# velocyto-team/velocyto.py

Hardware: AMD Instinct MI355X
Metric: cells/sec through knn_imputation->fit_slope->colDeltaCor, 50k cells x 30k genes (higher is better)
Workload: dtype f64

## Files before the change

### velocyto.py_amd/csrc/coldeltacor.hip

```cpp
#include <stdlib.h>
#include "common.h"
#ifndef VCY_EXP
#define VCY_EXP 0
#endif
#include <type_traits>

namespace vcy {

template <typename T> __device__ __forceinline__ T fast_sqrt(T x);
template <> __device__ __forceinline__ float fast_sqrt<float>(float x) { return __builtin_amdgcn_sqrtf(x); }
template <> __device__ __forceinline__ double fast_sqrt<double>(double x) { return sqrt(x); }
template <typename T> __device__ __forceinline__ T fast_log10(T x);
template <> __device__ __forceinline__ float fast_log10<float>(float x) { return __builtin_amdgcn_logf(x) * 0.30102999566398120f; }
template <> __device__ __forceinline__ double fast_log10<double>(double x) { return log10(x); }

template <typename T, int TR, int RULES> __device__ __forceinline__ T xform(T t, T psc)
{
    if (TR == VCY_LINEAR) return t;
    const T a = fabs(t) + psc;
    const T s = (TR == VCY_SQRT) ? fast_sqrt<T>(a) : fast_log10<T>(a);
    if (TR == VCY_SQRT && RULES != VCY_RULES_FULL)
        return (fabs(t) < T(1e-16)) ? T(0) : copysign(s, t);
    T r;
    if (TR == VCY_LOG10 && RULES == VCY_RULES_PARTIAL) r = (t >= T(0)) ? s : -s;
    else r = (t > T(0)) ? s : -s;
    return r;
}

template <> __device__ __forceinline__ float xform<float, VCY_SQRT, VCY_RULES_PARTIAL>(float t, float psc)
{
    const float c = __builtin_amdgcn_fmed3f(fabsf(t) * 0x1p54f, 0.0f, 1.0f);
    return copysignf(fast_sqrt<float>(fmaf(psc, c, fabsf(t))), t);
}

template <> __device__ __forceinline__ double xform<double, VCY_SQRT, VCY_RULES_PARTIAL_ROOT2>(double t, double psc)
{
    const double x = fabs(t) + psc;
    const float xf0 = (float)x;
    const float xf = (fabs(t) < 1e-16) ? __builtin_inff() : xf0;
    const float yf = __builtin_amdgcn_rsqf(xf);
    const double s0 = (double)(xf0 * yf), h = (double)(0.5f * yf);
    double d = fma(-s0, s0, x);
    const double s1 = fma(d, h, s0);
    d = fma(-s1, s1, x);
    return copysign(fma(d, h, s1), t);
}

template <> __device__ __forceinline__ double xform<double, VCY_SQRT, VCY_RULES_PARTIAL>(double t, double psc)
{
    const double x = fabs(t) + psc;
    const float xf0 = (float)x;
    const float xf = (fabs(t) < 1e-16) ? __builtin_inff() : xf0;
    const double y = (double)__builtin_amdgcn_rsqf(xf);
    const double u = x * y;
    return copysign(u * fma(-u, y, 3.0), t);
}

extern "C" __device__ float vcy_fmul_legacy(float, float) __asm("llvm.amdgcn.fmul.legacy");
template <> __device__ __forceinline__ float xform<float, VCY_SQRT, VCY_RULES_PARTIAL_NOPSC>(float t, float)
{
    return vcy_fmul_legacy(t, __builtin_amdgcn_rsqf(fabsf(t)));
}

template <int TR, int RULES> struct Shifted { static constexpr bool value = TR == VCY_LOG10 || (TR == VCY_SQRT && RULES == VCY_RULES_FULL); };

template <typename T, int TR, int RULES> struct ZeroMasked {
    static constexpr bool value = std::is_same<T, double>::value && TR == VCY_SQRT && (RULES == VCY_RULES_PARTIAL || RULES == VCY_RULES_PARTIAL_ROOT2);
};
template <int RULES> __device__ __forceinline__ double xform_kept(double t, double psc)
{
    const double x = fabs(t) + psc;
    const float xf = (float)x;
    const float yf = __builtin_amdgcn_rsqf(xf);
    if constexpr (RULES == VCY_RULES_PARTIAL_ROOT2) {
        const double s0 = (double)(xf * yf), h = (double)(0.5f * yf);
        double d = fma(-s0, s0, x);
        const double s1 = fma(d, h, s0);
        d = fma(-s1, s1, x);
        return copysign(fma(d, h, s1), t);
    } else {
        const double y = (double)yf;
        const double u = x * y;
        return copysign(u * fma(-u, y, 3.0), t);
    }
}

template <typename T, int TR, int RULES> __device__ __forceinline__ T xform_shift(T psc)
{
    if (!Shifted<TR, RULES>::value) return T(0);
    const T k = xform<T, TR, RULES>(T(0), psc);
    return (k - k == T(0)) ? k : T(0);
}
template <> __device__ __forceinline__ float xform_shift<float, VCY_LOG10, VCY_RULES_PARTIAL>(float psc)
{
    const float l0 = __builtin_amdgcn_logf(psc);
    return (l0 - l0 == 0.f) ? l0 : 0.f;
}
template <> __device__ __forceinline__ float xform_shift<float, VCY_LOG10, VCY_RULES_FULL>(float psc)
{
    const float l0 = -__builtin_amdgcn_logf(psc);
    return (l0 - l0 == 0.f) ? l0 : 0.f;
}

template <typename T, int TR, int RULES> __device__ __forceinline__ T xform_s(T t, T psc, T K)
{
    const T a = xform<T, TR, RULES>(t, psc);
    return Shifted<TR, RULES>::value ? a - K : a;
}
template <> __device__ __forceinline__ float xform_s<float, VCY_LOG10, VCY_RULES_PARTIAL>(float t, float psc, float K)
{
    const float l = __builtin_amdgcn_logf(fabsf(t) + psc);
    return (((t >= 0.f) ? l : -l) - K) * 0.30102999566398120f;
}
template <> __device__ __forceinline__ float xform_s<float, VCY_LOG10, VCY_RULES_FULL>(float t, float psc, float K)
{
    const float l = __builtin_amdgcn_logf(fabsf(t) + psc);
    return (((t > 0.f) ? l : -l) - K) * 0.30102999566398120f;
}

template <typename T> __device__ __forceinline__ T pearson_from_moments(double sA, double sAA, double sAb, double sb, double sbb, double n)
{
    if (n < 2.0) return (T)__builtin_nan("");
    const double cov = sAb - sA * sb / n;
    const double va = sAA - sA * sA / n;
    const double vb = sbb - sb * sb / n;
    return (T)(cov / sqrt(va * vb));
}

template <typename T> struct FuseArgs {
    const T *Ux;
    const float *gamma, *q;
    T dt_shift, used_dt;
};

template <typename T, int TR> __device__ __forceinline__ T fused_dmat(T s, T u, float gm, float qq, T dt_shift, T used_dt, T psc)
{
    const T upred = (T)gm * s + (T)qq;
    const T ds = dt_shift * (u - upred);
    const T D = (s + used_dt * ds) - s;
    if (TR == VCY_LINEAR) return D;
    const T a = fabs(D) + psc;
    const T f = (TR == VCY_SQRT) ? fast_sqrt<T>(a) : fast_log10<T>(a);
    return D > T(0) ? f : (D < T(0) ? -f : T(0) * f);
}

template <typename T, int TR, int RULES>
__global__ __launch_bounds__(1024) void k_cdc_partial(const T *__restrict__ e, const T *__restrict__ d,
                                                       const int32_t *__restrict__ ixs, T *__restrict__ out,
                                                       const int32_t *__restrict__ order, int G, int64_t ld,
                                                       int64_t cell0, int64_t d_row0, int C_out, int nrndm, int gchunk, T psc, FuseArgs<T> fuse)
{
    using V = typename Vec<T>::type;
    constexpr int N = Vec<T>::N;
    constexpr int UNROLL = 4;
    extern __shared__ __attribute__((aligned(16))) char smem[];
    T *ec = reinterpret_cast<T *>(smem);
    T *dc = ec + gchunk;
    T *acc = dc + gchunk;
    double *red = reinterpret_cast<double *>(acc + 3 * ((nrndm + 1) & ~1));

    const int tid = threadIdx.x, lane = tid & 63, wave = tid >> 6, nwaves = blockDim.x >> 6;
    const int per_x = (C_out + 7) / 8;
    const int pos = ((int)blockIdx.x & 7) * per_x + ((int)blockIdx.x >> 3);
    if (pos >= C_out) return;
    const int cl = order ? order[pos] : pos;
    const int64_t c = cell0 + cl;
    const T *erow_c = e + c * ld;
    const T *drow_c = (fuse.Ux ? fuse.Ux : d) + (c - d_row0) * ld;

    for (int n = tid; n < 3 * nrndm; n += blockDim.x) acc[n] = T(0);
    double sb = 0.0, sbb = 0.0;
    const T K = xform_shift<T, TR, RULES>(psc);

    for (int g0 = 0; g0 < G; g0 += gchunk) {
        const int gl = min(gchunk, G - g0);
        const int nvec = gl / N;
        __syncthreads();
        for (int v = tid; v < nvec; v += blockDim.x) {
            const V ev = reinterpret_cast<const V *>(erow_c + g0)[v];
            V dv = reinterpret_cast<const V *>(drow_c + g0)[v];
            if (fuse.Ux) {
                const T *ep = reinterpret_cast<const T *>(&ev);
                T *dq = reinterpret_cast<T *>(&dv);
#pragma unroll
                for (int k = 0; k < N; ++k) {
                    const int g = g0 + v * N + k;
                    dq[k] = fused_dmat<T, TR>(ep[k], dq[k], fuse.gamma[g], fuse.q ? fuse.q[g] : 0.f, fuse.dt_shift, fuse.used_dt, psc);
                }
            }
            reinterpret_cast<V *>(ec)[v] = ev;
            reinterpret_cast<V *>(dc)[v] = dv;
            const T *dp = reinterpret_cast<const T *>(&dv);
#pragma unroll
            for (int k = 0; k < N; ++k) { sb += (double)dp[k]; sbb += (double)dp[k] * (double)dp[k]; }
        }
        for (int g = nvec * N + tid; g < gl; g += blockDim.x) {
            const T ev = erow_c[g0 + g];
            T dv = drow_c[g0 + g];
            if (fuse.Ux) dv = fused_dmat<T, TR>(ev, dv, fuse.gamma[g0 + g], fuse.q ? fuse.q[g0 + g] : 0.f, fuse.dt_shift, fuse.used_dt, psc);
            ec[g] = ev; dc[g] = dv;
            sb += (double)dv; sbb += (double)dv * (double)dv;
        }
        __syncthreads();

        for (int n = wave; n < nrndm; n += nwaves) {
            const int i = __builtin_amdgcn_readfirstlane(ixs[(int64_t)cl * nrndm + n]);
            const T *row = e + (int64_t)i * ld + g0;
            T sA[N], sAA[N], sAb[N];
#pragma unroll
            for (int k = 0; k < N; ++k) { sA[k] = T(0); sAA[k] = T(0); sAb[k] = T(0); }
            int v = lane;
            for (; v + 64 * (UNROLL - 1) < nvec; v += 64 * UNROLL) {
                V x[UNROLL];
#pragma unroll
                for (int u = 0; u < UNROLL; ++u) x[u] = reinterpret_cast<const V *>(row)[v + 64 * u];
#pragma unroll
                for (int u = 0; u < UNROLL; ++u) {
                    const V ecv = reinterpret_cast<const V *>(ec)[v + 64 * u];
                    const V dcv = reinterpret_cast<const V *>(dc)[v + 64 * u];
                    const T *xp = reinterpret_cast<const T *>(&x[u]);
                    const T *ep = reinterpret_cast<const T *>(&ecv);
                    const T *bp = reinterpret_cast<const T *>(&dcv);
#pragma unroll
                    for (int k = 0; k < N; ++k) {
                        const T tt = xp[k] - ep[k];
                        T a = xform_s<T, TR, RULES>(tt, psc, K);
                        sA[k] += a;
                        if (RULES == VCY_RULES_PARTIAL_NOPSC) sAA[k] += fabs(tt);
                        else sAA[k] = fma(a, a, sAA[k]);
                        sAb[k] = fma(a, bp[k], sAb[k]);
                    }
                }
            }
            for (; v < nvec; v += 64) {
                const V xv = reinterpret_cast<const V *>(row)[v];
                const V ecv = reinterpret_cast<const V *>(ec)[v];
                const V dcv = reinterpret_cast<const V *>(dc)[v];
                const T *xp = reinterpret_cast<const T *>(&xv);
                const T *ep = reinterpret_cast<const T *>(&ecv);
                const T *bp = reinterpret_cast<const T *>(&dcv);
#pragma unroll
                for (int k = 0; k < N; ++k) {
                    const T tt = xp[k] - ep[k];
                    T a = xform_s<T, TR, RULES>(tt, psc, K);
                    sA[k] += a;
                    if (RULES == VCY_RULES_PARTIAL_NOPSC) sAA[k] += fabs(tt);
                    else sAA[k] = fma(a, a, sAA[k]);
                    sAb[k] = fma(a, bp[k], sAb[k]);
                }
            }
            {
                const int g = nvec * N + lane;
                if (g < gl) {
                    const T tt = row[g] - ec[g];
                    T a = xform_s<T, TR, RULES>(tt, psc, K);
                    sA[0] += a;
                    if (RULES == VCY_RULES_PARTIAL_NOPSC) sAA[0] += fabs(tt);
                    else sAA[0] = fma(a, a, sAA[0]);
                    sAb[0] = fma(a, dc[g], sAb[0]);
                }
            }
            T tA = sA[0], tAA = sAA[0], tAb = sAb[0];
#pragma unroll
            for (int k = 1; k < N; ++k) { tA += sA[k]; tAA += sAA[k]; tAb += sAb[k]; }
            tA = wave_sum(tA); tAA = wave_sum(tAA); tAb = wave_sum(tAb);
            if (lane == 0) {
                acc[3 * n + 0] += tA;
                acc[3 * n + 1] += tAA;
                acc[3 * n + 2] += tAb;
            }
        }
    }
    sb = block_sum(sb, red);
    sbb = block_sum(sbb, red);
    for (int n = tid; n < nrndm; n += blockDim.x)
        out[(int64_t)cl * nrndm + n] = pearson_from_moments<T>((double)acc[3 * n], (double)acc[3 * n + 1],
                                                               (double)acc[3 * n + 2], sb, sbb, (double)G);
}

constexpr int GRP_NV = 6;
constexpr int GRP_GC_DUAL = 6, GRP_NV_DUAL = 6;
constexpr int GRP_GC = 8;
constexpr int GRP_GC_F64 = 6, GRP_NV_F64 = 8;
constexpr int GRP_GC_DUAL_F64 = 4;

template <typename T> __host__ __device__ inline size_t grouped_lds_bytes(int gc, int nv, bool dual, int64_t maxpairs, int npad)
{
    const int as = dual ? 4 : 3;
    return (size_t)(dual ? 3 : 2) * gc * nv * 64 * 16 + (size_t)npad * 8 + sizeof(T) * (size_t)as * ((maxpairs + 1) & ~(int64_t)1) +
           8 * (size_t)(maxpairs + 2 > 64 + 4 * gc ? maxpairs + 2 : 64 + 4 * gc) + (size_t)(gc + 18) * sizeof(int) + 16;
}

template <int K, bool FULL> struct RowVecs { static constexpr int value = K; static constexpr bool full = FULL; };
template <int K, int NV, typename F> __device__ __forceinline__ void for_even_count(int n, F &f)
{
    if constexpr (K + 2 <= NV) {
        if (n == K) f(RowVecs<K, false>{});
        else for_even_count<K + 2, NV>(n, f);
    } else
        f(RowVecs<K, false>{});
}

template <typename T, int TR, int RULES, int GC, int NV, bool DUAL>
__global__ __launch_bounds__(1024) void k_cdc_partial_grouped(const T *__restrict__ e, const T *__restrict__ d, const T *__restrict__ d2,
                                                               const int32_t *__restrict__ ixs, T *__restrict__ out, T *__restrict__ out2,
                                                               const int32_t *__restrict__ order, int G, int64_t ld, int64_t cell0,
                                                               int64_t d_row0, int C_main, int tile_main, int C_tail, int tile_tail, int nrndm_all, int stride, int npad, T psc,
                                                               FuseArgs<T> fuse)
{
    using V = typename Vec<T>::type;
    constexpr int N = Vec<T>::N;
    constexpr int GCHUNK = NV * 64 * N;
    constexpr int AS = DUAL ? 4 : 3;
    constexpr int PW = DUAL ? 4 : 2;
    extern __shared__ __attribute__((aligned(16))) char smem[];
    const int maxpairs = GC * max(tile_main, tile_tail);
    T *ec = reinterpret_cast<T *>(smem);
    T *dc = ec + GC * GCHUNK;
    T *dc2 = dc + GC * GCHUNK;
    unsigned long long *keys = reinterpret_cast<unsigned long long *>(dc + (DUAL ? 2 : 1) * GC * GCHUNK);
    T *acc = reinterpret_cast<T *>(keys + npad);
    unsigned long long *desc = reinterpret_cast<unsigned long long *>(acc + AS * ((maxpairs + 1) & ~1));
    double *part = reinterpret_cast<double *>(desc);
    double *s_sb = part + 64, *s_sbb = s_sb + GC, *s_sb2 = s_sbb + GC, *s_sbb2 = s_sb2 + GC;
    int *s_cells = reinterpret_cast<int *>(desc + max(maxpairs + 2, 64 + 4 * GC));
    int *s_wavetot = s_cells + GC;
    int &s_U = s_wavetot[16];
    int *s_next = s_wavetot + 17;

    const int tid = threadIdx.x, lane = tid & 63, wave = tid >> 6, nwaves = blockDim.x >> 6;
    const int nb_main = ((((C_main + GC - 1) / GC) + 7) / 8 * 8) * (C_main > 0 ? (nrndm_all + tile_main - 1) / tile_main : 0);
    const bool tail = (int)blockIdx.x >= nb_main;
    const int bx = tail ? (int)blockIdx.x - nb_main : (int)blockIdx.x;
    const int C_out = tail ? C_tail : C_main, pos0 = tail ? C_main : 0, tilew = tail ? tile_tail : tile_main;
    const int ngroups = (C_out + GC - 1) / GC, per = (ngroups + 7) / 8, gblocks = per * 8;
    const int tile = bx / gblocks, bg = bx - tile * gblocks;
    const int gpos = (bg & 7) * per + (bg >> 3);
    if (gpos >= ngroups) return;
    const int n0 = tile * tilew;
    const int nrndm = min(tilew, nrndm_all - n0);
    ixs += n0;
    out += n0;
    if (DUAL) out2 += n0;
    const int g0cell = gpos * GC;
    const int gcount = min(GC, C_out - g0cell);
    const int npairs = gcount * nrndm;
    if (tid < GC) s_cells[tid] = tid < gcount ? (order ? order[pos0 + g0cell + tid] : pos0 + g0cell + tid) : 0;
    __syncthreads();
    for (int t = tid; t < npad; t += blockDim.x) {
        unsigned long long key = ~0ull;
        if (t < npairs) {
            const int m = t / nrndm, n = t - m * nrndm;
            const unsigned i = (unsigned)ixs[(int64_t)s_cells[m] * stride + n];
            key = ((unsigned long long)i << 16) | ((unsigned long long)m << 12) | (unsigned)n;
        }
        keys[t] = key;
    }
    __syncthreads();
    for (int size = 2; size <= npad; size <<= 1) {
        for (int stride = size >> 1; stride > 0; stride >>= 1) {
            for (int t = tid; t < npad / 2; t += blockDim.x) {
                const int lo = 2 * t - (t & (stride - 1)), hi = lo + stride;
                const bool up = ((lo & size) == 0);
                const unsigned long long a = keys[lo], b = keys[hi];
                if ((a > b) == up) { keys[lo] = b; keys[hi] = a; }
            }
            __syncthreads();
        }
    }
    {
        static_assert(GC <= 8, "member mask is 8 bits");
        auto head = [&](int t) {
            if (t == 0) return true;
            const unsigned long long a = keys[t] >> 12, b = keys[t - 1] >> 12;
            return (a >> 4) != (b >> 4) || a == b;
        };
        const int per = (npad + blockDim.x - 1) / blockDim.x;
        const int t0 = tid * per, t1 = min(npairs, t0 + per);
        int cnt = 0;
        for (int t = t0; t < t1; ++t) cnt += head(t) ? 1 : 0;
        int incl = cnt;
#pragma unroll
        for (int off = 1; off < 64; off <<= 1) { const int o = __shfl_up(incl, off, 64); if (lane >= off) incl += o; }
        if (lane == 63) s_wavetot[wave] = incl;
        __syncthreads();
        int base = 0;
        for (int w = 0; w < wave; ++w) base += s_wavetot[w];
        int rank = base + incl - cnt;
        for (int t = t0; t < t1; ++t)
            if (head(t)) {
                unsigned mask = 0;
                int q = t;
                do { mask |= 1u << (unsigned)((keys[q] >> 12) & 15); ++q; } while (q < npairs && !head(q));
                desc[rank++] = ((keys[t] >> 16) << 19) | ((unsigned long long)mask << 11) | (unsigned)t;
            }
        if (tid == blockDim.x - 1) { s_U = base + incl; }
        __syncthreads();
    }
    for (int t = tid; t < AS * npairs; t += blockDim.x) acc[t] = T(0);
    __syncthreads();
    const int U = s_U;
    const T K = xform_shift<T, TR, RULES>(psc);
    const int sm = wave % GC, sh = wave / GC, snh = max(1, nwaves / GC);
    double psb = 0.0, psbb = 0.0, psb2 = 0.0, psbb2 = 0.0;

    for (int g0 = 0; g0 < G; g0 += GCHUNK) {
        const int gl = min(GCHUNK, G - g0);
        const int nvec = (gl + N - 1) / N;
        const bool ragged = (gl % N) != 0;
        const int nvu = min(NV, ((nvec + 63) / 64 + 1) & ~1);
        __syncthreads();
        if (tid == 0) *s_next = 0;
        if (sh < snh && sm < gcount) {
            const int64_t c = cell0 + s_cells[sm];
            const T *er = e + c * ld + g0;
            const T *dr = (fuse.Ux ? fuse.Ux : d) + (c - d_row0) * ld + g0;
            const T *dr2 = DUAL ? d2 + (c - d_row0) * ld + g0 : nullptr;
            for (int v = sh * 64 + lane; v < nvec; v += 64 * snh) {
                V ev = reinterpret_cast<const V *>(er)[v];
                V dv = reinterpret_cast<const V *>(dr)[v];
                V dv2;
                if (DUAL) dv2 = reinterpret_cast<const V *>(dr2)[v];
                T *dp = reinterpret_cast<T *>(&dv);
                T *dp2 = reinterpret_cast<T *>(&dv2);
                T *ep = reinterpret_cast<T *>(&ev);
                if (fuse.Ux) {
#pragma unroll
                    for (int k = 0; k < N; ++k) {
                        const int g = g0 + v * N + k;
                        if (g < G) dp[k] = fused_dmat<T, TR>(ep[k], dp[k], fuse.gamma[g], fuse.q ? fuse.q[g] : 0.f, fuse.dt_shift, fuse.used_dt, psc);
                    }
                }
                if (ragged && v == nvec - 1) {
#pragma unroll
                    for (int k = 0; k < N; ++k) if (k >= gl - v * N) { dp[k] = T(0); ep[k] = T(0); if (DUAL) dp2[k] = T(0); }
                }
                reinterpret_cast<V *>(ec + sm * GCHUNK)[v] = ev;
                reinterpret_cast<V *>(dc + sm * GCHUNK)[v] = dv;
                if (DUAL) reinterpret_cast<V *>(dc2 + sm * GCHUNK)[v] = dv2;
#pragma unroll
                for (int k = 0; k < N; ++k) {
                    psb += (double)dp[k]; psbb += (double)dp[k] * (double)dp[k];
                    if (DUAL) { psb2 += (double)dp2[k]; psbb2 += (double)dp2[k] * (double)dp2[k]; }
                }
            }
        }
        if (gl < GCHUNK && sh < snh && sm < gcount)
            for (int v = nvec + sh * 64 + lane; v < nvu * 64; v += 64 * snh) {
                reinterpret_cast<V *>(ec + sm * GCHUNK)[v] = V{};
                reinterpret_cast<V *>(dc + sm * GCHUNK)[v] = V{};
                if (DUAL) reinterpret_cast<V *>(dc2 + sm * GCHUNK)[v] = V{};
            }
        __syncthreads();
        static_assert(NV % 2 == 0, "operand buffers alternate");
#define VCY_FENCE() __builtin_amdgcn_sched_barrier(0)
        auto load_row = [&](auto nvc, V (&x)[NV], unsigned long long dsc) {
            constexpr int KV = decltype(nvc)::value;
            const T *row = e + (int64_t)(dsc >> 19) * ld + g0;
#pragma unroll
            for (int u = 0; u < KV; ++u) {
                const int v = lane + 64 * u;
                if (decltype(nvc)::full || v < nvec) x[u] = reinterpret_cast<const V *>(row)[v];
                else x[u] = V{};
            }
        };
        auto eval_row = [&](auto nvc, const V (&x)[NV], unsigned long long dsc) {
            constexpr int KV = decltype(nvc)::value;
            int p = (int)(dsc & 2047);
            unsigned mask = (unsigned)(dsc >> 11) & 255u;
            int m = __builtin_ctz(mask);
            constexpr int RD = 2;
            static_assert(KV % RD == 0, "operand buffers rotate");
            V eR[RD], bR[RD], b2R[RD];
            auto rd = [&](V &ev, V &bv, V &b2v, int mm, int u) {
                ev = reinterpret_cast<const V *>(ec + mm * GCHUNK)[lane + 64 * u];
                bv = reinterpret_cast<const V *>(dc + mm * GCHUNK)[lane + 64 * u];
                if (DUAL) b2v = reinterpret_cast<const V *>(dc2 + mm * GCHUNK)[lane + 64 * u];
            };
#pragma unroll
            for (int u = 0; u < RD - 1; ++u) rd(eR[u], bR[u], b2R[u], m, u);
            while (mask) {
                mask &= mask - 1;
                const int mn = mask ? __builtin_ctz(mask) : m;
                T sA, sAA, sAb, sAb2;
                constexpr bool MASKED = ZeroMasked<T, TR, RULES>::value;
                if constexpr (MASKED) { sA = sAA = sAb = T(0); if (DUAL) sAb2 = T(0); }
                auto fold = [&](const V &xv, const V &ev, const V &bv, const V &b2v, bool first) {
                    const T *xp = reinterpret_cast<const T *>(&xv);
                    const T *ep = reinterpret_cast<const T *>(&ev);
                    const T *bp = reinterpret_cast<const T *>(&bv);
                    const T *bp2 = reinterpret_cast<const T *>(&b2v);
                    constexpr bool ABS2 = RULES == VCY_RULES_PARTIAL_NOPSC;
#pragma unroll
                    for (int k = 0; k < N; ++k) {
                        const T tt = xp[k] - ep[k];
                        if constexpr (MASKED) {
                            if (!(fabs(tt) < 1e-16)) {
                                const T a = xform_kept<RULES>(tt, psc);
                                sA += a;
                                sAA = fma(a, a, sAA);
                                sAb = fma(a, bp[k], sAb);
                                if (DUAL) sAb2 = fma(a, bp2[k], sAb2);
                            }
                            continue;
                        }
                        const T a = xform_s<T, TR, RULES>(tt, psc, K);
                        if (first && k == 0) {
                            sA = a;
                            sAA = ABS2 ? fabs(tt) : a * a;
                            sAb = a * bp[k];
                            if (DUAL) sAb2 = a * bp2[k];
                            continue;
                        }
                        sA += a;
                        if (ABS2) sAA += fabs(tt);
                        else sAA = fma(a, a, sAA);
                        sAb = fma(a, bp[k], sAb);
                        if (DUAL) sAb2 = fma(a, bp2[k], sAb2);
                    }
                };
#pragma unroll
                for (int u = 0; u < KV; ++u) {
                    constexpr int AHEAD = RD - 1;
                    const int un = u + AHEAD;
                    if (un < KV) rd(eR[un % RD], bR[un % RD], b2R[un % RD], m, un);
                    else rd(eR[un % RD], bR[un % RD], b2R[un % RD], mn, un - KV);
                    VCY_FENCE();
                    fold(x[u], eR[u % RD], bR[u % RD], b2R[u % RD], u == 0);
                    VCY_FENCE();
                }
                const T tot = wave_sum_rows_quads(sA, sAA, sAb, DUAL ? sAb2 : T(0));
                if ((lane & 3) == 0 && (lane >> 4) < AS)
                    __hip_atomic_fetch_add(&acc[AS * p + (lane >> 4)], tot, __ATOMIC_RELAXED, __HIP_MEMORY_SCOPE_WORKGROUP);
                ++p;
                m = mn;
            }
        };
        auto rows = [&](auto nvc) {
            auto ticket = [&]() { int t = 0; if (lane == 0) t = atomicAdd(s_next, 1); return t; };
            auto uni = [&](unsigned long long v) {
                const unsigned lo = (unsigned)__builtin_amdgcn_readfirstlane((int)(unsigned)v);
                const unsigned hi = (unsigned)__builtin_amdgcn_readfirstlane((int)(unsigned)(v >> 32));
                return ((unsigned long long)hi << 32) | lo;
            };
            constexpr int TAIL = 64;
            const int U4 = U > TAIL ? ((U - TAIL) & ~3) : 0, T4 = U4 >> 2;
            auto first_row = [&](int v) { return v < T4 ? 4 * v : U4 + 2 * (v - T4); };
            V xa[NV], xb[NV];
            int v = __builtin_amdgcn_readfirstlane(ticket());
            int q = min(first_row(v), U);
            unsigned long long w0 = 0, w1 = 0, w2 = 0, w3 = 0;
            if (q < U) { w0 = uni(desc[q]); w1 = uni(desc[min(q + 1, U - 1)]); w2 = uni(desc[min(q + 2, U - 1)]); w3 = uni(desc[min(q + 3, U - 1)]); }
            if (q < U) load_row(nvc, xa, w0);
            while (v < T4) {
                const int tv = ticket();
                load_row(nvc, xb, w1);
                eval_row(nvc, xa, w0);
                load_row(nvc, xa, w2);
                eval_row(nvc, xb, w1);
                const int vn = __builtin_amdgcn_readfirstlane(tv);
                const int qn = min(first_row(vn), U);
                unsigned long long n0 = 0, n1 = 0, n2 = 0, n3 = 0;
                if (qn < U) { n0 = desc[qn]; n1 = desc[min(qn + 1, U - 1)]; n2 = desc[min(qn + 2, U - 1)]; n3 = desc[min(qn + 3, U - 1)]; }
                load_row(nvc, xb, w3);
                eval_row(nvc, xa, w2);
                if (qn < U) { n0 = uni(n0); n1 = uni(n1); n2 = uni(n2); n3 = uni(n3); }
                if (qn < U) load_row(nvc, xa, n0);
                eval_row(nvc, xb, w3);
                v = vn; q = qn; w0 = n0; w1 = n1; w2 = n2; w3 = n3;
            }
            while (q < U) {
                const int tv = ticket();
                const bool two = q + 1 < U;
                if (two) load_row(nvc, xb, w1);
                eval_row(nvc, xa, w0);
                const int vn = __builtin_amdgcn_readfirstlane(tv);
                const int qn = min(first_row(vn), U);
                unsigned long long n0 = 0, n1 = 0;
                if (qn < U) { n0 = uni(desc[qn]); n1 = uni(desc[min(qn + 1, U - 1)]); }
                if (qn < U) load_row(nvc, xa, n0);
                if (two) eval_row(nvc, xb, w1);
                v = vn; q = qn; w0 = n0; w1 = n1;
            }
        };
        if (nvec == 64 * NV) rows(RowVecs<NV, true>{});
        else for_even_count<2, NV>(nvu, rows);
    }
    psb = wave_sum(psb); psbb = wave_sum(psbb);
    if (DUAL) { psb2 = wave_sum(psb2); psbb2 = wave_sum(psbb2); }
    __syncthreads();
    if (lane == 0) {
        part[PW * wave] = psb; part[PW * wave + 1] = psbb;
        if (DUAL) { part[PW * wave + 2] = psb2; part[PW * wave + 3] = psbb2; }
    }
    __syncthreads();
    if (tid < gcount) {
        double a = 0.0, b = 0.0, a2 = 0.0, b2 = 0.0;
        for (int h = 0; h < snh; ++h) {
            const int w = tid + h * GC;
            if (w < nwaves) { a += part[PW * w]; b += part[PW * w + 1]; if (DUAL) { a2 += part[PW * w + 2]; b2 += part[PW * w + 3]; } }
        }
        s_sb[tid] = a; s_sbb[tid] = b; s_sb2[tid] = a2; s_sbb2[tid] = b2;
    }
    __syncthreads();
    for (int p = tid; p < npairs; p += blockDim.x) {
        const unsigned long long key = keys[p];
        const int m = (int)((key >> 12) & 15), n = (int)(key & 4095);
        const double mA = (double)acc[AS * p], mAA = (double)acc[AS * p + 1];
        out[(int64_t)s_cells[m] * stride + n] = pearson_from_moments<T>(mA, mAA, (double)acc[AS * p + 2], s_sb[m], s_sbb[m], (double)G);
        if (DUAL) out2[(int64_t)s_cells[m] * stride + n] = pearson_from_moments<T>(mA, mAA, (double)acc[AS * p + 3], s_sb2[m], s_sbb2[m], (double)G);
    }
}

constexpr int FULL_TC = 16, FULL_TI = 64, FULL_GK = 32;

template <typename T, int TR>
__global__ __launch_bounds__(256) void k_cdc_full(const T *__restrict__ e, const T *__restrict__ d, T *__restrict__ rm,
                                                   int C, int G, int64_t ld, int64_t cell0, int C_out, int64_t ld_rm,
                                                   T psc, int accumulate)
{
    __shared__ T ei[FULL_TI][FULL_GK + 1];
    __shared__ T ecs[FULL_TC][FULL_GK];
    __shared__ T dcs[FULL_TC][FULL_GK];
    __shared__ double sbs[FULL_TC][2];
    const int tid = threadIdx.x, il = tid & 63, cg = tid >> 6;
    const int i0 = blockIdx.x * FULL_TI, c0 = blockIdx.y * FULL_TC;
    T sA[4], sAA[4], sAb[4];
#pragma unroll
    for (int k = 0; k < 4; ++k) { sA[k] = T(0); sAA[k] = T(0); sAb[k] = T(0); }
    const int sg = tid & 31, sr = tid >> 5;
    double sb = 0.0, sbb = 0.0;
    double sb2 = 0.0, sbb2 = 0.0;
    const T K = xform_shift<T, TR, VCY_RULES_FULL>(psc);
    for (int g0 = 0; g0 < G; g0 += FULL_GK) {
        const int glen = min(FULL_GK, G - g0);
        __syncthreads();
        const bool gok = sg < glen;
#pragma unroll
        for (int r = 0; r < 8; ++r) {
            const int row = sr + 8 * r, gi = i0 + row;
            ei[row][sg] = (gok && gi < C) ? e[(int64_t)gi * ld + g0 + sg] : T(0);
        }
#pragma unroll
        for (int r = 0; r < 2; ++r) {
            const int row = sr + 8 * r;
            const int64_t gc = cell0 + c0 + row;
            const bool ok = gok && (c0 + row) < C_out;
            const T ev = ok ? e[gc * ld + g0 + sg] : T(0);
            const T dv = ok ? d[gc * ld + g0 + sg] : T(0);
            ecs[row][sg] = ev;
            dcs[row][sg] = dv;
            if (r == 0) { sb += (double)dv; sbb += (double)dv * (double)dv; }
            else { sb2 += (double)dv; sbb2 += (double)dv * (double)dv; }
        }
        __syncthreads();
        for (int g = 0; g < glen; ++g) {
            const T x = ei[il][g];
#pragma unroll
            for (int k = 0; k < 4; ++k) {
                T a = xform_s<T, TR, VCY_RULES_FULL>(x - ecs[cg * 4 + k][g], psc, K);
                sA[k] += a;
                sAA[k] = fma(a, a, sAA[k]);
                sAb[k] = fma(a, dcs[cg * 4 + k][g], sAb[k]);
            }
        }
    }
#pragma unroll
    for (int off = 16; off > 0; off >>= 1) {
        sb += __shfl_xor(sb, off, 64); sbb += __shfl_xor(sbb, off, 64);
        sb2 += __shfl_xor(sb2, off, 64); sbb2 += __shfl_xor(sbb2, off, 64);
    }
    if (sg == 0) { sbs[sr][0] = sb; sbs[sr][1] = sbb; sbs[sr + 8][0] = sb2; sbs[sr + 8][1] = sbb2; }
    __syncthreads();
    const int gi = i0 + il;
    if (gi < C) {
#pragma unroll
        for (int k = 0; k < 4; ++k) {
            const int crow = c0 + cg * 4 + k;
            if (crow < C_out) {
                const T r = pearson_from_moments<T>((double)sA[k], (double)sAA[k], (double)sAb[k],
                                                    sbs[cg * 4 + k][0], sbs[cg * 4 + k][1], (double)G);
                T *p = rm + (int64_t)crow * ld_rm + gi;
                *p = accumulate ? (*p + r) : r;
            }
        }
    }
}

template <typename T>
__global__ void k_scatter_rows(const T *__restrict__ vals, const int32_t *__restrict__ ixs, T *__restrict__ rm,
                               int64_t total, int nrndm, int64_t ld_rm)
{
    for (int64_t t = blockIdx.x * (int64_t)blockDim.x + threadIdx.x; t < total; t += (int64_t)gridDim.x * blockDim.x) {
        const int64_t c = t / nrndm;
        atomicAdd(rm + c * ld_rm + ixs[t], vals[t]);
    }
}

template <typename T, int TR, int RULES, int GC, int NV, bool DUAL>
static int launch_grouped(const void *e, const void *d, const void *d2, const int32_t *ixs, void *out, void *out2, const int32_t *order, int64_t G,
                          int64_t ld, int64_t cell0, int64_t C_out, int64_t d_row0, int64_t nrndm, double psc, hipStream_t st,
                          FuseArgs<T> fuse, const DevInfo &dev, bool *done)
{
    constexpr int64_t TILE_MAX = 256;
    static_assert(GC * TILE_MAX <= 2048, "a row descriptor holds the first pair of the row in 11 bits");
    *done = false;
    const size_t budget_g = (size_t)(dev.lds_optin > 163840 ? 163840 : dev.lds_optin);
    int64_t ntiles = (nrndm + TILE_MAX - 1) / TILE_MAX, tile = 0;
    int npad = 2;
    size_t lds_g = 0;
    for (;; ++ntiles) {
        tile = (nrndm + ntiles - 1) / ntiles;
        const int64_t maxpairs = GC * tile;
        for (npad = 2; npad < maxpairs; npad <<= 1) {}
        lds_g = grouped_lds_bytes<T>(GC, NV, DUAL, maxpairs, npad);
        if (lds_g <= budget_g || tile <= 16) break;
    }
    if (!(nrndm >= 8 && C_out >= 4 * GC && nrndm <= 0x7fffffff / 2 && lds_g <= budget_g)) return VCY_OK;
    auto kern = k_cdc_partial_grouped<T, TR, RULES, GC, NV, DUAL>;
    int rc = ensure_dynamic_lds(reinterpret_cast<const void *>(kern), lds_g);
    if (rc) return rc;
    const int64_t groups = (C_out + GC - 1) / GC, W = dev.cus > 0 ? dev.cus : 256;
    const int64_t full = groups >= W ? groups / W * W : 0;
    const int64_t c_main = full * GC, c_tail = C_out - c_main;
    int64_t tw = tile;
    if (c_tail > 0) {
        const int64_t left = groups - full;
        constexpr double OVH = 0.05;
        double best = 0.0;
        int64_t bs = 1;
        for (int64_t s = 1; s == 1 || (tile + s - 1) / s >= 16; ++s) {
            const int64_t w = (tile + s - 1) / s, nt = (nrndm + w - 1) / w;
            const double t = (double)((left * nt + W - 1) / W) * ((double)w / (double)tile + OVH);
            if (s == 1 || t < 0.98 * best) { best = t; bs = s; }
        }
        tw = (tile + bs - 1) / bs;
    }
    auto nblocks = [&](int64_t ncell, int64_t w) { return ncell > 0 ? ((ncell + GC - 1) / GC + 7) / 8 * 8 * ((nrndm + w - 1) / w) : (int64_t)0; };
    hipLaunchKernelGGL(kern, dim3((unsigned)(nblocks(c_main, tile) + nblocks(c_tail, tw))), dim3(1024), lds_g, st, (const T *)e, (const T *)d,
                       (const T *)d2, ixs, (T *)out, (T *)out2, order, (int)G, ld, cell0, d_row0, (int)c_main, (int)tile, (int)c_tail, (int)tw,
                       (int)nrndm, (int)nrndm, npad, (T)psc, fuse);
    VCY_LAUNCH_CHECK();
    *done = true;
    return VCY_OK;
}

template <typename T, int TR, int RULES>
static int launch_partial(const void *e, const void *d, const void *d2, const int32_t *ixs, void *out, void *out2, const int32_t *order, int64_t G,
                          int64_t ld, int64_t cell0, int64_t C_out, int64_t d_row0, int64_t nrndm, double psc, hipStream_t st,
                          FuseArgs<T> fuse = FuseArgs<T>{nullptr, nullptr, nullptr, T(1), T(1)})
{
    constexpr int N = Vec<T>::N;
    DevInfo dev;
    int rc = device_info(&dev);
    if (rc) return rc;
    if (env_int("VCY_CDC_GROUP", GRP_GC) == GRP_GC) {
        bool done = false;
        if (d2) {
            if constexpr (sizeof(T) == 8) {
                if (env_int("VCY_CDC_DUAL_F64", 1) == 1)
                    rc = launch_grouped<T, TR, RULES, GRP_GC_DUAL_F64, GRP_NV_F64, true>(e, d, d2, ixs, out, out2, order, G, ld, cell0, C_out, d_row0, nrndm, psc, st, fuse, dev, &done);
                else
                    rc = launch_grouped<T, TR, RULES, GRP_GC_DUAL, GRP_NV_DUAL, true>(e, d, d2, ixs, out, out2, order, G, ld, cell0, C_out, d_row0, nrndm, psc, st, fuse, dev, &done);
            } else
                rc = launch_grouped<T, TR, RULES, GRP_GC_DUAL, GRP_NV_DUAL, true>(e, d, d2, ixs, out, out2, order, G, ld, cell0, C_out, d_row0, nrndm, psc, st, fuse, dev, &done);
        } else if constexpr (sizeof(T) == 8)
            rc = launch_grouped<T, TR, RULES, GRP_GC_F64, GRP_NV_F64, false>(e, d, nullptr, ixs, out, nullptr, order, G, ld, cell0, C_out, d_row0, nrndm, psc, st, fuse, dev, &done);
        else
            rc = launch_grouped<T, TR, RULES, GRP_GC, GRP_NV, false>(e, d, nullptr, ixs, out, nullptr, order, G, ld, cell0, C_out, d_row0, nrndm, psc, st, fuse, dev, &done);
        if (rc || done) return rc;
    }
    if (d2) {
        rc = launch_partial<T, TR, RULES>(e, d, nullptr, ixs, out, nullptr, order, G, ld, cell0, C_out, d_row0, nrndm, psc, st, fuse);
        if (rc) return rc;
        return launch_partial<T, TR, RULES>(e, d2, nullptr, ixs, out2, nullptr, order, G, ld, cell0, C_out, d_row0, nrndm, psc, st);
    }
    const int quantum = 64 * N;
    const size_t fixed = sizeof(T) * 3 * ((nrndm + 1) & ~1) + 32 * sizeof(double);
    const size_t budget = (size_t)(dev.lds_optin > 153600 ? 153600 : dev.lds_optin);
    if (fixed + 2 * quantum * sizeof(T) > budget)
        return fail(VCY_ERR_UNSUPPORTED, "%s: nrndm=%lld needs more LDS than the %lld-byte budget", "coldeltacor_partial", (long long)nrndm, (long long)budget);
    const int64_t max_chunk = (int64_t)((budget - fixed) / (2 * sizeof(T))) / quantum * quantum;
    const int64_t Gq = (G + quantum - 1) / quantum * quantum;
    const int64_t nchunks = (Gq + max_chunk - 1) / max_chunk;
    int64_t gchunk = ((Gq / quantum + nchunks - 1) / nchunks) * quantum;
    const size_t lds = fixed + 2 * gchunk * sizeof(T);
    auto kern = k_cdc_partial<T, TR, RULES>;
    rc = ensure_dynamic_lds(reinterpret_cast<const void *>(kern), lds);
    if (rc) return rc;
    const int threads = (nrndm >= 16) ? 1024 : (nrndm >= 8 ? 512 : 256);
    hipLaunchKernelGGL(kern, dim3((unsigned)((C_out + 7) / 8 * 8)), dim3(threads), lds, st, (const T *)e, (const T *)d, ixs, (T *)out, order,
                       (int)G, ld, cell0, d_row0, (int)C_out, (int)nrndm, (int)gchunk, (T)psc, fuse);
    VCY_LAUNCH_CHECK();
    return VCY_OK;
}

template <typename T>
static int dispatch_partial(const void *e, const void *d, const void *d2, const int32_t *ixs, void *out, void *out2, const int32_t *order, int64_t G,
                            int64_t ld, int64_t cell0, int64_t C_out, int64_t d_row0, int64_t nrndm, int transform, int rules,
                            double psc, hipStream_t st, FuseArgs<T> fuse = FuseArgs<T>{nullptr, nullptr, nullptr, T(1), T(1)})
{
#define VCY_CASE(TR, RU) \
    if (transform == TR && rules == RU) return launch_partial<T, TR, RU>(e, d, d2, ixs, out, out2, order, G, ld, cell0, C_out, d_row0, nrndm, psc, st, fuse);
    if (rules == VCY_RULES_PARTIAL_ROOT2) {
        if constexpr (std::is_same<T, double>::value) { VCY_CASE(VCY_SQRT, VCY_RULES_PARTIAL_ROOT2) }
        rules = VCY_RULES_PARTIAL;
    }
    VCY_CASE(VCY_LINEAR, VCY_RULES_PARTIAL)
    VCY_CASE(VCY_LINEAR, VCY_RULES_FULL)
    VCY_CASE(VCY_SQRT, VCY_RULES_PARTIAL)
    VCY_CASE(VCY_SQRT, VCY_RULES_FULL)
    VCY_CASE(VCY_LOG10, VCY_RULES_PARTIAL)
    VCY_CASE(VCY_LOG10, VCY_RULES_FULL)
    if constexpr (std::is_same<T, float>::value) { VCY_CASE(VCY_SQRT, VCY_RULES_PARTIAL_NOPSC) }
#undef VCY_CASE
    if (rules == VCY_RULES_PARTIAL_NOPSC) return fail(VCY_ERR_INVALID, "%s: VCY_RULES_PARTIAL_NOPSC is defined for VCY_SQRT on VCY_F32 only", "coldeltacor_partial");
    return fail(VCY_ERR_INVALID, "%s: bad transform/rules", "coldeltacor_partial");
}

template <typename T>
static int dispatch_full(const void *e, const void *d, void *rm, int64_t C, int64_t G, int64_t ld, int64_t cell0,
                         int64_t C_out, int64_t ld_rm, int transform, double psc, int accumulate, hipStream_t st)
{
    dim3 grid((unsigned)((C + FULL_TI - 1) / FULL_TI), (unsigned)((C_out + FULL_TC - 1) / FULL_TC));
#define VCY_CASE(TR)                                                                                                        \
    if (transform == TR) {                                                                                                  \
        hipLaunchKernelGGL((k_cdc_full<T, TR>), grid, dim3(256), 0, st, (const T *)e, (const T *)d, (T *)rm, (int)C, (int)G, \
                           ld, cell0, (int)C_out, ld_rm, (T)psc, accumulate);                                              \
        VCY_LAUNCH_CHECK();                                                                                                 \
        return VCY_OK;                                                                                                      \
    }
    VCY_CASE(VCY_LINEAR)
    VCY_CASE(VCY_SQRT)
    VCY_CASE(VCY_LOG10)
#undef VCY_CASE
    return fail(VCY_ERR_INVALID, "%s: bad transform", "coldeltacor_full");
}

}

using namespace vcy;

static int check_partial_args(const char *who, const void *e, const void *d, const int32_t *ixs, const void *out, int64_t C, int64_t G, int64_t ld,
                              int64_t cell0, int64_t C_out, int64_t d_row0, int64_t nrndm, int dtype)
{
    if (!(e && d && ixs && out)) return fail(VCY_ERR_INVALID, "%s: null pointer", who);
    if (!(C > 0 && G > 0 && nrndm > 0 && C_out > 0 && cell0 >= 0 && cell0 + C_out <= C)) return fail(VCY_ERR_INVALID, "%s: bad shape", who);
    if (ld < G) return fail(VCY_ERR_INVALID, "%s: ld < G", who);
    if (!(d_row0 >= 0 && d_row0 <= cell0)) return fail(VCY_ERR_INVALID, "%s: d must cover cells cell0..cell0+C_out-1", who);
    if (!(dtype == VCY_F32 || dtype == VCY_F64)) return fail(VCY_ERR_INVALID, "%s: bad dtype", who);
    if (ld % (dtype == VCY_F32 ? 4 : 2) != 0) return fail(VCY_ERR_INVALID, "%s: ld must keep rows 16-byte aligned", who);
    if (((uintptr_t)e % 16) || ((uintptr_t)d % 16)) return fail(VCY_ERR_INVALID, "%s: e/d must be 16-byte aligned", who);
    return VCY_OK;
}

extern "C" int vcy_coldeltacor_partial(const void *e, const void *d, const int32_t *ixs, void *out, const int32_t *order,
                                       int64_t C, int64_t G, int64_t ld, int64_t cell0, int64_t C_out, int64_t d_row0,
                                       int64_t nrndm, int transform, int rules, double psc, int dtype, vcy_stream stream)
{
    int rc = check_partial_args("coldeltacor_partial", e, d, ixs, out, C, G, ld, cell0, C_out, d_row0, nrndm, dtype);
    if (rc) return rc;
    hipStream_t st = as_stream(stream);
    if (dtype == VCY_F32) return dispatch_partial<float>(e, d, nullptr, ixs, out, nullptr, order, G, ld, cell0, C_out, d_row0, nrndm, transform, rules, psc, st);
    return dispatch_partial<double>(e, d, nullptr, ixs, out, nullptr, order, G, ld, cell0, C_out, d_row0, nrndm, transform, rules, psc, st);
}

extern "C" int vcy_coldeltacor_partial_dual(const void *e, const void *d, const void *d_rndm, const int32_t *ixs, void *out, void *out_rndm,
                                            const int32_t *order, int64_t C, int64_t G, int64_t ld, int64_t cell0, int64_t C_out, int64_t d_row0,
                                            int64_t nrndm, int transform, int rules, double psc, int dtype, vcy_stream stream)
{
    int rc = check_partial_args("coldeltacor_partial_dual", e, d, ixs, out, C, G, ld, cell0, C_out, d_row0, nrndm, dtype);
    if (rc) return rc;
    VCY_REQUIRE(d_rndm && out_rndm && out_rndm != out, "coldeltacor_partial_dual: d_rndm / out_rndm missing");
    VCY_REQUIRE((uintptr_t)d_rndm % 16 == 0, "coldeltacor_partial_dual: d_rndm must be 16-byte aligned");
    hipStream_t st = as_stream(stream);
    if (dtype == VCY_F32) return dispatch_partial<float>(e, d, d_rndm, ixs, out, out_rndm, order, G, ld, cell0, C_out, d_row0, nrndm, transform, rules, psc, st);
    return dispatch_partial<double>(e, d, d_rndm, ixs, out, out_rndm, order, G, ld, cell0, C_out, d_row0, nrndm, transform, rules, psc, st);
}

extern "C" int vcy_coldeltacor_partial_fused(const void *Sx_sz, const void *Ux_sz, const float *gamma, const float *q, const int32_t *ixs,
                                            void *out, const int32_t *order, int64_t C, int64_t G, int64_t ld, int64_t cell0, int64_t C_out,
                                            int64_t u_row0, int64_t nrndm, int transform, int rules, double psc, double dt_shift,
                                            double used_dt, int dtype, vcy_stream stream)
{
    int rc = check_partial_args("coldeltacor_partial_fused", Sx_sz, Ux_sz, ixs, out, C, G, ld, cell0, C_out, u_row0, nrndm, dtype);
    if (rc) return rc;
    VCY_REQUIRE(gamma, "coldeltacor_partial_fused: null pointer");
    hipStream_t st = as_stream(stream);
    if (dtype == VCY_F32) {
        FuseArgs<float> f{(const float *)Ux_sz, gamma, q, (float)dt_shift, (float)used_dt};
        return dispatch_partial<float>(Sx_sz, Ux_sz, nullptr, ixs, out, nullptr, order, G, ld, cell0, C_out, u_row0, nrndm, transform, rules, psc, st, f);
    }
    FuseArgs<double> f{(const double *)Ux_sz, gamma, q, dt_shift, used_dt};
    return dispatch_partial<double>(Sx_sz, Ux_sz, nullptr, ixs, out, nullptr, order, G, ld, cell0, C_out, u_row0, nrndm, transform, rules, psc, st, f);
}

extern "C" int vcy_coldeltacor_partial_fused_dual(const void *Sx_sz, const void *Ux_sz, const float *gamma, const float *q, const void *d_rndm,
                                                 const int32_t *ixs, void *out, void *out_rndm, const int32_t *order, int64_t C, int64_t G, int64_t ld,
                                                 int64_t cell0, int64_t C_out, int64_t u_row0, int64_t nrndm, int transform, int rules, double psc,
                                                 double dt_shift, double used_dt, int dtype, vcy_stream stream)
{
    int rc = check_partial_args("coldeltacor_partial_fused_dual", Sx_sz, Ux_sz, ixs, out, C, G, ld, cell0, C_out, u_row0, nrndm, dtype);
    if (rc) return rc;
    VCY_REQUIRE(gamma && d_rndm && out_rndm && out_rndm != out, "coldeltacor_partial_fused_dual: null pointer");
    VCY_REQUIRE((uintptr_t)d_rndm % 16 == 0, "coldeltacor_partial_fused_dual: d_rndm must be 16-byte aligned");
    hipStream_t st = as_stream(stream);
    if (dtype == VCY_F32) {
        FuseArgs<float> f{(const float *)Ux_sz, gamma, q, (float)dt_shift, (float)used_dt};
        return dispatch_partial<float>(Sx_sz, Ux_sz, d_rndm, ixs, out, out_rndm, order, G, ld, cell0, C_out, u_row0, nrndm, transform, rules, psc, st, f);
    }
    FuseArgs<double> f{(const double *)Ux_sz, gamma, q, dt_shift, used_dt};
    return dispatch_partial<double>(Sx_sz, Ux_sz, d_rndm, ixs, out, out_rndm, order, G, ld, cell0, C_out, u_row0, nrndm, transform, rules, psc, st, f);
}

extern "C" int vcy_coldeltacor_full(const void *e, const void *d, void *rm, int64_t C, int64_t G, int64_t ld, int64_t cell0,
                                    int64_t C_out, int64_t ld_rm, int transform, double psc, int accumulate, int dtype,
                                    vcy_stream stream)
{
    VCY_REQUIRE(e && d && rm, "coldeltacor_full: null pointer");
    VCY_REQUIRE(C > 0 && G > 0 && C_out > 0 && cell0 >= 0 && cell0 + C_out <= C && ld >= G && ld_rm >= C, "coldeltacor_full: bad shape");
    VCY_REQUIRE(dtype == VCY_F32 || dtype == VCY_F64, "coldeltacor_full: bad dtype");
    hipStream_t st = as_stream(stream);
    if (dtype == VCY_F32) return dispatch_full<float>(e, d, rm, C, G, ld, cell0, C_out, ld_rm, transform, psc, accumulate, st);
    return dispatch_full<double>(e, d, rm, C, G, ld, cell0, C_out, ld_rm, transform, psc, accumulate, st);
}

extern "C" int vcy_scatter_rows(const void *vals, const int32_t *ixs, void *rm, int64_t C_out, int64_t nrndm, int64_t ld_rm,
                                int dtype, vcy_stream stream)
{
    VCY_REQUIRE(vals && ixs && rm && C_out > 0 && nrndm > 0, "scatter_rows: bad arguments");
    const int64_t total = C_out * nrndm;
    const int blocks = (int)((total + 255) / 256 > 4096 ? 4096 : (total + 255) / 256);
    hipStream_t st = as_stream(stream);
    if (dtype == VCY_F32) hipLaunchKernelGGL(k_scatter_rows<float>, dim3(blocks), dim3(256), 0, st, (const float *)vals, ixs, (float *)rm, total, (int)nrndm, ld_rm);
    else if (dtype == VCY_F64) hipLaunchKernelGGL(k_scatter_rows<double>, dim3(blocks), dim3(256), 0, st, (const double *)vals, ixs, (double *)rm, total, (int)nrndm, ld_rm);
    else return fail(VCY_ERR_INVALID, "%s: bad dtype", "scatter_rows");
    VCY_LAUNCH_CHECK();
    return VCY_OK;
}
```

Before: 227,300.

## Make grouped colDeltaCor kernel persistent with per-XCD atomic work queues and stealing

Turns the grouped partial kernel into a persistent kernel that launches about one block per CU. Each block takes work units from one of eight per-XCD atomic queue heads chosen by the hardware XCD id, and steals from the queue with the most work left once its own queue is empty. Kernel arguments are packed into a struct and re-read through the kernarg pointer on every loop iteration to limit register pressure. The aim is better load balance and cache locality per XCD, at the cost of an extra memset, atomics per unit, and a lazily allocated queue buffer per stream.

```diff
diff --git a/velocyto.py_amd/csrc/coldeltacor.hip b/velocyto.py_amd/csrc/coldeltacor.hip
--- a/velocyto.py_amd/csrc/coldeltacor.hip
+++ b/velocyto.py_amd/csrc/coldeltacor.hip
@@ -3,7 +3,10 @@
 #ifndef VCY_EXP
 #define VCY_EXP 0
 #endif
+#include <map>
+#include <mutex>
 #include <type_traits>
+#include <utility>
 
 namespace vcy {
 
@@ -288,7 +291,7 @@
 {
     const int as = dual ? 4 : 3;
     return (size_t)(dual ? 3 : 2) * gc * nv * 64 * 16 + (size_t)npad * 8 + sizeof(T) * (size_t)as * ((maxpairs + 1) & ~(int64_t)1) +
-           8 * (size_t)(maxpairs + 2 > 64 + 4 * gc ? maxpairs + 2 : 64 + 4 * gc) + (size_t)(gc + 18) * sizeof(int) + 16;
+           8 * (size_t)(maxpairs + 2 > 64 + 4 * gc ? maxpairs + 2 : 64 + 4 * gc) + (size_t)(gc + 19) * sizeof(int) + 16;
 }
 
 template <int K, bool FULL> struct RowVecs { static constexpr int value = K; static constexpr bool full = FULL; };
@@ -301,12 +304,20 @@
         f(RowVecs<K, false>{});
 }
 
+template <typename T> struct GroupedArgs {
+    const T *e, *d, *d2;
+    const int32_t *ixs;
+    T *out, *out2;
+    const int32_t *order;
+    unsigned *queue;
+    int64_t ld, cell0, d_row0;
+    int G, C_main, tile_main, C_tail, tile_tail, nrndm_all, stride, npad, nunits;
+    T psc;
+    FuseArgs<T> fuse;
+};
+
 template <typename T, int TR, int RULES, int GC, int NV, bool DUAL>
-__global__ __launch_bounds__(1024) void k_cdc_partial_grouped(const T *__restrict__ e, const T *__restrict__ d, const T *__restrict__ d2,
-                                                               const int32_t *__restrict__ ixs, T *__restrict__ out, T *__restrict__ out2,
-                                                               const int32_t *__restrict__ order, int G, int64_t ld, int64_t cell0,
-                                                               int64_t d_row0, int C_main, int tile_main, int C_tail, int tile_tail, int nrndm_all, int stride, int npad, T psc,
-                                                               FuseArgs<T> fuse)
+__global__ __launch_bounds__(1024) void k_cdc_partial_grouped(GroupedArgs<T>)
 {
     using V = typename Vec<T>::type;
     constexpr int N = Vec<T>::N;
@@ -314,6 +325,21 @@
     constexpr int AS = DUAL ? 4 : 3;
     constexpr int PW = DUAL ? 4 : 2;
     extern __shared__ __attribute__((aligned(16))) char smem[];
+    typedef const GroupedArgs<T> __attribute__((address_space(4))) *ArgPtr;
+    ArgPtr ka = (ArgPtr)__builtin_amdgcn_kernarg_segment_ptr();
+  for (;;) {
+    int tid = threadIdx.x, nthr = blockDim.x;
+    asm volatile("" : "+s"(ka), "+v"(tid), "+s"(nthr));
+    const int lane = tid & 63, wave = tid >> 6, nwaves = nthr >> 6;
+    const T *__restrict__ e = ka->e, *__restrict__ d = ka->d, *__restrict__ d2 = ka->d2;
+    const int32_t *__restrict__ ixs_all = ka->ixs, *__restrict__ order = ka->order;
+    T *__restrict__ out_all = ka->out, *__restrict__ out2_all = ka->out2;
+    unsigned *__restrict__ queue = ka->queue;
+    const int64_t ld = ka->ld, cell0 = ka->cell0, d_row0 = ka->d_row0;
+    const int G = ka->G, C_main = ka->C_main, tile_main = ka->tile_main, C_tail = ka->C_tail, tile_tail = ka->tile_tail;
+    const int nrndm_all = ka->nrndm_all, stride = ka->stride, npad = ka->npad;
+    const T psc = ka->psc;
+    const FuseArgs<T> fuse{ka->fuse.Ux, ka->fuse.gamma, ka->fuse.q, ka->fuse.dt_shift, ka->fuse.used_dt};
     const int maxpairs = GC * max(tile_main, tile_tail);
     T *ec = reinterpret_cast<T *>(smem);
     T *dc = ec + GC * GCHUNK;
@@ -327,27 +353,51 @@
     int *s_wavetot = s_cells + GC;
     int &s_U = s_wavetot[16];
     int *s_next = s_wavetot + 17;
-
-    const int tid = threadIdx.x, lane = tid & 63, wave = tid >> 6, nwaves = blockDim.x >> 6;
+    int *s_unit = s_wavetot + 18;
+
     const int nb_main = ((((C_main + GC - 1) / GC) + 7) / 8 * 8) * (C_main > 0 ? (nrndm_all + tile_main - 1) / tile_main : 0);
-    const bool tail = (int)blockIdx.x >= nb_main;
-    const int bx = tail ? (int)blockIdx.x - nb_main : (int)blockIdx.x;
+    const int xcd = (int)(__builtin_amdgcn_s_getreg(20 | (3 << 11)) & 7u);
+    const int qlen = ka->nunits >> 3;
+    __syncthreads();
+    if (tid == 0) {
+        int u = -1;
+        unsigned q = __hip_atomic_fetch_add(&queue[xcd], 1u, __ATOMIC_RELAXED, __HIP_MEMORY_SCOPE_AGENT);
+        if (q < (unsigned)qlen) u = 8 * (int)q + xcd;
+        else
+            for (;;) {
+                int best = -1, left = 0;
+                for (int y = 0; y < 8; ++y) {
+                    const unsigned h = __hip_atomic_load(&queue[y], __ATOMIC_RELAXED, __HIP_MEMORY_SCOPE_AGENT);
+                    const int l = h < (unsigned)qlen ? qlen - (int)h : 0;
+                    if (l > left) { left = l; best = y; }
+                }
+                if (best < 0) break;
+                q = __hip_atomic_fetch_add(&queue[best], 1u, __ATOMIC_RELAXED, __HIP_MEMORY_SCOPE_AGENT);
+                if (q < (unsigned)qlen) { u = 8 * (int)q + best; break; }
+            }
+        *s_unit = u;
+    }
+    __syncthreads();
+    const int unit = *s_unit;
+    if (unit < 0) break;
+    const bool tail = unit >= nb_main;
+    const int bx = tail ? unit - nb_main : unit;
     const int C_out = tail ? C_tail : C_main, pos0 = tail ? C_main : 0, tilew = tail ? tile_tail : tile_main;
     const int ngroups = (C_out + GC - 1) / GC, per = (ngroups + 7) / 8, gblocks = per * 8;
     const int tile = bx / gblocks, bg = bx - tile * gblocks;
     const int gpos = (bg & 7) * per + (bg >> 3);
-    if (gpos >= ngroups) return;
+    if (gpos >= ngroups) continue;
     const int n0 = tile * tilew;
     const int nrndm = min(tilew, nrndm_all - n0);
-    ixs += n0;
-    out += n0;
-    if (DUAL) out2 += n0;
+    const int32_t *__restrict__ ixs = ixs_all + n0;
+    T *__restrict__ out = out_all + n0;
+    T *__restrict__ out2 = DUAL ? out2_all + n0 : nullptr;
     const int g0cell = gpos * GC;
     const int gcount = min(GC, C_out - g0cell);
     const int npairs = gcount * nrndm;
     if (tid < GC) s_cells[tid] = tid < gcount ? (order ? order[pos0 + g0cell + tid] : pos0 + g0cell + tid) : 0;
     __syncthreads();
-    for (int t = tid; t < npad; t += blockDim.x) {
+    for (int t = tid; t < npad; t += nthr) {
         unsigned long long key = ~0ull;
         if (t < npairs) {
             const int m = t / nrndm, n = t - m * nrndm;
@@ -359,7 +409,7 @@
     __syncthreads();
     for (int size = 2; size <= npad; size <<= 1) {
         for (int stride = size >> 1; stride > 0; stride >>= 1) {
-            for (int t = tid; t < npad / 2; t += blockDim.x) {
+            for (int t = tid; t < npad / 2; t += nthr) {
                 const int lo = 2 * t - (t & (stride - 1)), hi = lo + stride;
                 const bool up = ((lo & size) == 0);
                 const unsigned long long a = keys[lo], b = keys[hi];
@@ -375,7 +425,7 @@
             const unsigned long long a = keys[t] >> 12, b = keys[t - 1] >> 12;
             return (a >> 4) != (b >> 4) || a == b;
         };
-        const int per = (npad + blockDim.x - 1) / blockDim.x;
+        const int per = (npad + nthr - 1) / nthr;
         const int t0 = tid * per, t1 = min(npairs, t0 + per);
         int cnt = 0;
         for (int t = t0; t < t1; ++t) cnt += head(t) ? 1 : 0;
@@ -394,10 +444,10 @@
                 do { mask |= 1u << (unsigned)((keys[q] >> 12) & 15); ++q; } while (q < npairs && !head(q));
                 desc[rank++] = ((keys[t] >> 16) << 19) | ((unsigned long long)mask << 11) | (unsigned)t;
             }
-        if (tid == blockDim.x - 1) { s_U = base + incl; }
+        if (tid == nthr - 1) { s_U = base + incl; }
         __syncthreads();
     }
-    for (int t = tid; t < AS * npairs; t += blockDim.x) acc[t] = T(0);
+    for (int t = tid; t < AS * npairs; t += nthr) acc[t] = T(0);
     __syncthreads();
     const int U = s_U;
     const T K = xform_shift<T, TR, RULES>(psc);
@@ -603,13 +653,14 @@
         s_sb[tid] = a; s_sbb[tid] = b; s_sb2[tid] = a2; s_sbb2[tid] = b2;
     }
     __syncthreads();
-    for (int p = tid; p < npairs; p += blockDim.x) {
+    for (int p = tid; p < npairs; p += nthr) {
         const unsigned long long key = keys[p];
         const int m = (int)((key >> 12) & 15), n = (int)(key & 4095);
         const double mA = (double)acc[AS * p], mAA = (double)acc[AS * p + 1];
         out[(int64_t)s_cells[m] * stride + n] = pearson_from_moments<T>(mA, mAA, (double)acc[AS * p + 2], s_sb[m], s_sbb[m], (double)G);
         if (DUAL) out2[(int64_t)s_cells[m] * stride + n] = pearson_from_moments<T>(mA, mAA, (double)acc[AS * p + 3], s_sb2[m], s_sbb2[m], (double)G);
     }
+  }
 }
 
 constexpr int FULL_TC = 16, FULL_TI = 64, FULL_GK = 32;
@@ -695,6 +746,23 @@
         const int64_t c = t / nrndm;
         atomicAdd(rm + c * ld_rm + ixs[t], vals[t]);
     }
+}
+
+static int queue_heads(hipStream_t st, unsigned **out)
+{
+    static std::mutex mutex;
+    static std::map<std::pair<int, hipStream_t>, unsigned *> heads;
+    int dev = 0;
+    VCY_CHECK_HIP(hipGetDevice(&dev));
+    std::lock_guard<std::mutex> lock(mutex);
+    unsigned *&p = heads[std::make_pair(dev, st)];
+    if (!p) {
+        void *mem = nullptr;
+        VCY_CHECK_HIP(hipMalloc(&mem, 256));
+        p = static_cast<unsigned *>(mem);
+    }
+    *out = p;
+    return VCY_OK;
 }
 
 template <typename T, int TR, int RULES, int GC, int NV, bool DUAL>
@@ -737,9 +805,15 @@
         tw = (tile + bs - 1) / bs;
     }
     auto nblocks = [&](int64_t ncell, int64_t w) { return ncell > 0 ? ((ncell + GC - 1) / GC + 7) / 8 * 8 * ((nrndm + w - 1) / w) : (int64_t)0; };
-    hipLaunchKernelGGL(kern, dim3((unsigned)(nblocks(c_main, tile) + nblocks(c_tail, tw))), dim3(1024), lds_g, st, (const T *)e, (const T *)d,
-                       (const T *)d2, ixs, (T *)out, (T *)out2, order, (int)G, ld, cell0, d_row0, (int)c_main, (int)tile, (int)c_tail, (int)tw,
-                       (int)nrndm, (int)nrndm, npad, (T)psc, fuse);
+    const int64_t nunits = nblocks(c_main, tile) + nblocks(c_tail, tw);
+    if (nunits > 0x7fffffff) return VCY_OK;
+    unsigned *queue = nullptr;
+    rc = queue_heads(st, &queue);
+    if (rc) return rc;
+    VCY_CHECK_HIP(hipMemsetAsync(queue, 0, 8 * sizeof(unsigned), st));
+    GroupedArgs<T> ga{(const T *)e, (const T *)d, (const T *)d2, ixs, (T *)out, (T *)out2, order, queue, ld, cell0, d_row0, (int)G, (int)c_main, (int)tile,
+                      (int)c_tail, (int)tw, (int)nrndm, (int)nrndm, npad, (int)nunits, (T)psc, fuse};
+    hipLaunchKernelGGL(kern, dim3((unsigned)(nunits < W ? nunits : W)), dim3(1024), lds_g, st, ga);
     VCY_LAUNCH_CHECK();
     *done = true;
     return VCY_OK;
```

Measured after the change: 232,200, median of 6. 1.02x the previous value.
